# google-deepmind/mujoco_mpc

Measured on NVIDIA H100. Metric: env-steps/sec, higher is better.
Workload: dtype f32

## Files before the change

### mujoco_mpc_b200/csrc/dev_data.cuh

```cuda
#pragma once
#include <cuda_runtime.h>

#include "dev_model.h"

#ifndef MJPC_NO_COMPACT
#define MJPC_COMPACT 1
#endif
#ifdef MJPC_COMPACT
#define MJPC_ROLL _Pragma("unroll 1")
#define MJPC_HESS_ROLLED 1
#else
#define MJPC_ROLL
#endif

namespace mjpc_dev {

constexpr int kMaxSplinePoints = 64;
#define MJPC_D_ARRAYS(X)                                                                                          \
  X(qpos, M.nq) X(qvel, M.nv) X(ctrl, M.nu) X(qacc, M.nv) X(qacc_warmstart, M.nv) X(mocap_pos, 3 * M.nmocap)      \
  X(mocap_quat, 4 * M.nmocap) X(xpos, 3 * M.nbody) X(xquat, 4 * M.nbody) X(xmat, 9 * M.nbody)                     \
  X(xipos, 3 * M.nbody) X(ximat, 9 * M.nbody) X(xanchor, 3 * M.njnt) X(xaxis, 3 * M.njnt)                         \
  X(geom_xpos, 3 * M.ngeom) X(geom_xmat, 9 * M.ngeom) X(site_xpos, 3 * M.nsite) X(subtree_com, 3 * M.nbody)       \
  X(cinert, 10 * M.nbody) X(crb, 10 * M.nbody) X(cdof, 6 * M.nv) X(cdof_dot, 6 * M.nv) X(cvel, 6 * M.nbody)       \
  X(cacc, 6 * M.nbody) X(cfrc, 6 * M.nbody) X(cfrc_sub, 6 * M.nbody) X(subtree_linvel, 3 * M.nbody)               \
// ... 348 lines not shown
    y = mask_pick3(yj, lane == j, y - scaled * yj, lane > j, y, lane < j);
#pragma unroll
    for (int k = j + 1; k < N; k++) {
      const float lkj = __shfl_sync(kFull, row[j], k);
      row[k] -= row[j] * lkj;
    }
  }
  if (lane < N) {
#pragma unroll
    for (int k = 0; k < N; k++)
      if (k <= lane) A[lane * N + k] = row[k];
  }
  __syncwarp();
#pragma unroll
  for (int i = N - 1; i >= 0; i--) {
    const float xi = __shfl_sync(kFull, y, i) * il[i];
    if (lane == i) y = xi;
    if (lane < i) y -= A[i * N + lane] * xi;
  }
  if (lane < N) x[lane] = y;
  __syncwarp();
}

template <int N>
__device__ __forceinline__ void warp_chol_factor_solve_rolled(float* A, float* inv, float* x, const float* b, int lane) {
  const int li = lane < N ? lane : N - 1;
  float y = b[li];
  __syncwarp();
  float* rowi = A + li * N;
#pragma unroll 1
  for (int j = 0; j < N; j++) {
    const float* rowj = A + j * N;
    float s = rowi[j];
    int k = 0;
    if (N % 2 == 0) {
#pragma unroll 2
      for (; k + 1 < j; k += 2) {
        const float2 a = *reinterpret_cast<const float2*>(rowi + k), bb = *reinterpret_cast<const float2*>(rowj + k);
        s -= a.x * bb.x; s -= a.y * bb.y;
      }
    }
#pragma unroll 1
    for (; k < j; k++) s -= rowi[k] * rowj[k];
    float p = __shfl_sync(kFull, s, j);
    if (p < kMinVal) p = kMinVal;
    const float l = sqrtf(p), il = 1.0f / l;
    if (lane >= j && lane < N) rowi[j] = (lane == j) ? l : s * il;
    if (lane == j) inv[j] = il;
    __syncwarp();
  }
#pragma unroll 1
  for (int i = 0; i < N; i++) {
    const float yi = __shfl_sync(kFull, y, i) * inv[i];
    const float lij = rowi[i];
    y = (lane == i) ? yi : (lane > i ? y - lij * yi : y);
  }
#pragma unroll 1
  for (int i = N - 1; i >= 0; i--) {
    const float xi = __shfl_sync(kFull, y, i) * inv[i];
    const float lji = A[i * N + li];
    y = (lane == i) ? xi : (lane < i ? y - lji * xi : y);
  }
  if (lane < N) x[lane] = y;
  __syncwarp();
}

template <int NS>
__device__ __noinline__ void warp_chol_factor_solve(float* A, float* inv, float* x, const float* b, int n, int lane) {
#ifdef MJPC_CHOL_ROLLED2
  if constexpr (NS > 0 && NS <= 32) { warp_chol_factor_solve_rolled<NS>(A, inv, x, b, lane); return; }
  if (n == 18) { warp_chol_factor_solve_rolled<18>(A, inv, x, b, lane); return; }
#endif
#ifndef MJPC_CHOL_ROLLED
  if constexpr (NS > 0 && NS <= 32) { warp_chol_factor_solve_reg<NS>(A, x, b, lane); return; }
  if (n == 18) { warp_chol_factor_solve_reg<18>(A, x, b, lane); return; }
  if (n == 2) { warp_chol_factor_solve_reg<2>(A, x, b, lane); return; }
#endif
  warp_chol(A, inv, n, lane);
  warp_chol_solve(x, A, inv, b, n, lane);
}
#endif

}
```

### mujoco_mpc_b200/csrc/dev_model.h

```cpp
#pragma once
#include <cstdint>
#include <cstring>
#include <stdexcept>
#include <string>
#include <vector>

namespace mjpc_dev {

#define MJPC_F_ARRAYS(X)                                                                                         \
  X(body_pos) X(body_quat) X(body_ipos) X(body_iquat) X(body_mass) X(body_inertia) X(body_subtreemass)           \
  X(body_invweight0) X(jnt_pos) X(jnt_axis) X(jnt_range) X(jnt_stiffness) X(jnt_margin) X(jnt_solref)            \
  X(jnt_solimp) X(qpos0) X(qpos_spring) X(dof_damping) X(dof_armature) X(dof_frictionloss) X(dof_solref)         \
  X(dof_solimp) X(dof_invweight0) X(geom_size) X(geom_pos) X(geom_quat) X(geom_friction) X(geom_solmix)          \
  X(geom_solref) X(geom_solimp) X(geom_margin) X(geom_gap) X(geom_rbound) X(site_pos) X(site_quat)               \
  X(actuator_gear) X(actuator_gainprm) X(actuator_biasprm) X(actuator_ctrlrange) X(actuator_forcerange)          \
  X(key_qpos) X(task_weight) X(task_norm_parameter) X(task_parameters) X(task_state) X(wrap_coef) X(tendon_range)     \
  X(tendon_margin) X(tendon_solref) X(tendon_solimp) X(tendon_invweight0)
#define MJPC_I_ARRAYS(X)                                                                                         \
  X(body_parentid) X(body_rootid) X(body_jntnum) X(body_jntadr) X(body_dofnum) X(body_dofadr) X(body_mocapid)    \
  X(jnt_type) X(jnt_qposadr) X(jnt_dofadr) X(jnt_bodyid) X(jnt_limited) X(dof_bodyid) X(dof_jntid)               \
  X(dof_parentid) X(geom_type) X(geom_bodyid) X(geom_condim) X(geom_priority) X(site_bodyid) X(actuator_trnid) X(actuator_trntype)  \
  X(actuator_biastype) X(actuator_ctrllimited) X(actuator_forcelimited) X(pair_geom1) X(pair_geom2)              \
  X(ray_geoms) X(task_dim_norm_residual) X(task_norm) X(task_num_norm_parameter) X(task_trace_objtype)           \
  X(task_trace_objid) X(task_ids) X(tendon_adr) X(tendon_num) X(tendon_limited) X(wrap_dof) X(wrap_qposadr)
// ... 7 lines not shown
#undef X
      F_COUNT
};
enum IntArrayId {
#define X(n) I_##n,
  MJPC_I_ARRAYS(X) MJPC_I_DERIVED(X)
#undef X
      I_COUNT
};

enum { GEOM_PLANE = 0, GEOM_HFIELD, GEOM_SPHERE, GEOM_CAPSULE, GEOM_ELLIPSOID, GEOM_CYLINDER, GEOM_BOX };
enum { JNT_FREE = 0, JNT_BALL, JNT_SLIDE, JNT_HINGE };
enum { OBJ_BODY = 0, OBJ_XBODY, OBJ_GEOM, OBJ_SITE };
enum { CONE_PYRAMIDAL = 0, CONE_ELLIPTIC = 1 };
enum { RESIDUAL_PARTICLE = 0, RESIDUAL_PARTICLE_COPY = 1, RESIDUAL_CARTPOLE = 2, RESIDUAL_QUADRUPED_FLAT = 3,
       RESIDUAL_HUMANOID_STAND = 4, RESIDUAL_HUMANOID_TRACK = 5, RESIDUAL_SHADOW_REORIENT = 6 };

#define MJPC_M_INTS(X)                                                                                           \
  X(nq) X(nv) X(nu) X(nbody) X(njnt) X(ngeom) X(nsite) X(nmocap) X(nkey) X(npair) X(nray) X(nlevel) X(nmpair)    \
  X(ntendon)                                                                                                     \
  X(nfloss) X(nlimit) X(nhpair) X(cone) X(iterations) X(ls_iterations) X(disable_contact) X(disable_eulerdamp)  \
  X(disable_frictionloss) X(disable_limit) X(disable_refsafe) X(disable_warmstart) X(maxcon) X(maxefc)           \
  X(residual_id) X(num_residual) X(num_term) X(num_trace) X(num_parameters) X(task_state_size) X(any_damping)    \
  X(nf) X(ni)

struct DevModel {
#define X(n) int n;
  MJPC_M_INTS(X)
#undef X
  float timestep, impratio, tolerance, ls_tolerance, meaninertia, risk;
  float differentiable;
  float gravity[3];
  int fo[F_COUNT];
  int io[I_COUNT];
};

struct Blob {
  const uint8_t* p;
  size_t n;
  int nent;
  Blob(const void* data, size_t nbytes) : p((const uint8_t*)data), n(nbytes), nent(0) {
    if (!data || nbytes < 16 || std::memcmp(p, "MJPCB200", 8) != 0) throw std::runtime_error("bad model blob magic");
    std::memcpy(&nent, p + 12, 4);
    if ((size_t)16 + 56 * (size_t)nent > nbytes) throw std::runtime_error("truncated model blob");
  }
  bool find(const char* name, int* dt, int* cnt, int64_t* off) const {
    for (int i = 0; i < nent; i++) {
// ... 131 lines not shown
    std::vector<int> hi_, hj_, frow(nv, -1);
    for (int r = 0; r < nv; r++) for (int c2 = 0; c2 <= r; c2++) if (pat[(size_t)r * nv + c2]) { hi_.push_back(r); hj_.push_back(c2); }
    for (size_t k = 0; k < fl.size(); k++) frow[fl[k]] = (int)k;
    M.nhpair = (int)hi_.size();
    put(I_hpair_i, hi_); put(I_hpair_j, hj_); put(I_floss_row, frow);
    std::vector<int> cadr(nb, 0), cnum(nb, 0), cdofs;
    for (int bb = 0; bb < nb; bb++) {
      std::vector<int> ch;
      for (int d = lastdof[bb]; d >= 0; d = dofpar[d]) ch.push_back(d);
      cadr[bb] = (int)cdofs.size(); cnum[bb] = (int)ch.size();
      cdofs.insert(cdofs.end(), ch.rbegin(), ch.rend());
    }
    int widest = 0;
    for (size_t k = 0; k < g1.size(); k++) {
      const uint64_t c1 = chain(gb[g1[k]]), c2m = chain(gb[g2[k]]);
      const uint64_t mm = (c1 && c2m) ? (c1 ^ c2m) : (c1 | c2m);
      int cnt = 0;
      for (int r = 0; r < nv; r++) cnt += (int)((mm >> r) & 1);
      widest = std::max(widest, cnt);
    }
    if (widest > 16) throw std::runtime_error("a contact pair couples more than 16 dofs (compact Jacobian width)");
    put(I_chain_adr, cadr); put(I_chain_num, cnum); put(I_chain_dof, cdofs);
  }
  while (P.i.size() % 4) P.i.push_back(0);
  while (P.f.size() % 4) P.f.push_back(0.f);
  M.nf = (int)P.f.size(); M.ni = (int)P.i.size();
  return P;
}

}
```

### mujoco_mpc_b200/csrc/dev_physics.cuh

```cuda
#pragma once
#include "dev_data.cuh"

namespace mjpc_dev {



template <class SP>
__device__ __noinline__ void k_kinematics(Ctx& c) {
  auto&& M = SP::model(c);
  const int lane = c.lane;
  float *xpos = DF(xpos), *xquat = DF(xquat), *xmat = DF(xmat), *xipos = DF(xipos), *ximat = DF(ximat);
  float *xanchor = DF(xanchor), *xaxis = DF(xaxis);
  const float* qpos = DF(qpos);
  if (lane < 3) { xpos[lane] = 0; xipos[lane] = 0; }
  if (lane < 4) xquat[lane] = lane == 0 ? 1.f : 0.f;
  if (lane < 9) { float v = (lane % 4 == 0) ? 1.f : 0.f; xmat[lane] = v; ximat[lane] = v; }
  __syncwarp();
  const int *level_adr = MI(level_adr), *level_body = MI(level_body), *parentid = MI(body_parentid),
            *mocapid = MI(body_mocapid), *jntadr = MI(body_jntadr), *jntnum = MI(body_jntnum),
            *jtype = MI(jnt_type), *jqadr = MI(jnt_qposadr);
  const float *bpos = MF(body_pos), *bquat = MF(body_quat), *bipos = MF(body_ipos), *biquat = MF(body_iquat),
              *jpos = MF(jnt_pos), *jaxis = MF(jnt_axis), *qpos0 = MF(qpos0);
  for (int l = 0; l < M.nlevel; l++) {
    const int a = level_adr[l], e = level_adr[l + 1];
// ... 1014 lines not shown
  }
  __syncwarp();
  float* smooth = DF(qfrc_smooth);
  for (int i = lane; i < nv; i += 32) smooth[i] = passive[i] - bias[i] + qact[i];
  if (c.xfrc_on) {
    const float *xf = DF(xfrc), *cdof = DF(cdof), *xipos = DF(xipos), *scom = DF(subtree_com);
    const int *dbody = MI(dof_bodyid), *subend = MI(body_subtreeend), *rootid = MI(body_rootid);
    for (int i = lane; i < nv; i += 32) {
      const int b0 = dbody[i];
      const float* cd = cdof + 6 * i;
      float a = 0.f;
      MJPC_ROLL
      for (int b = b0; b < subend[b0]; b++) {
        float off[3], t[3];
        for (int q = 0; q < 3; q++) off[q] = xipos[3 * b + q] - scom[3 * rootid[b] + q];
        cross3(t, cd, off);
        const float* f = xf + 6 * b;
        for (int q = 0; q < 3; q++) a += (cd[3 + q] + t[q]) * f[q] + cd[q] * f[3 + q];
      }
      smooth[i] += a;
    }
  }
  __syncwarp();
  warp_chol_factor_solve<SP::kNV>(DF(qLD), DF(ldinv), DF(qacc_smooth), smooth, nv, lane);
}

template <class SP>
__device__ __noinline__ void k_reference(Ctx& c) {
  const int lane = c.lane;
  const float *qvel = DF(qvel), *K = DF(efc_K), *B = DF(efc_B), *imp = DF(efc_imp), *pos = DF(efc_pos),
              *margin = DF(efc_margin);
  float* aref = DF(efc_aref);
  const int nsimple = SP::model(c).nfloss + c.nlim;
  for (int i = lane; i < c.nefc; i += 32) {
    const float v = row_dot<SP>(c, i, nsimple, qvel);
    aref[i] = -B[i] * v - K[i] * imp[i] * (pos[i] - margin[i]);
  }
  __syncwarp();
}

template <class SP>
__device__ __noinline__ float k_update_constraint(Ctx& c, bool hess) {
  auto&& M = SP::model(c);
  const int lane = c.lane, nv = M.nv;
  const float *jar = DF(efc_jar), *D = DF(efc_D), *R = DF(efc_R), *floss = DF(efc_floss), *J = DF(efc_J);
  float *force = DF(efc_force), *X = DF(efc_W), *hw = DF(efc_hw), *xw = DF(efc_hc);
  int *state = DI(efc_state);
// ... 768 lines not shown
      const int i = min(b0 + lane, nv - 1);
      const bool on = b0 + lane < nv;
      const float a = Ma[i] - smooth[i] - qfc[i];
      if (on) grad[i] = a;
      g2 += on ? a * a : 0.f;
      const float m = fabsf(Ma[i]) + fabsf(smooth[i]) + fabsf(qfc[i]);
      ga += on ? m * m : 0.f;
    }
    const float gnorm2 = warp_sum(g2), gabs2 = warp_sum(ga);
    __syncwarp();
    if (iter > 0) {
      const float improvement = (old - cost) / scale_inv, gradient = sqrtf(gnorm2) / scale_inv;
      const float gfloor = kGradFloor * 1.1920929e-7f * sqrtf(gabs2) / scale_inv;
      if (gradient < fmaxf(tol, gfloor)) break;
      const bool resolvable = fabsf(old - cost) > 16.f * 1.1920929e-7f * fabsf(cost);
      if (resolvable) { if (improvement < tol) break; stalls = 0; }
      else if (gradient > 0.5f * prev_gradient && (alpha > 0.5f || ++stalls >= 3)) break;
      prev_gradient = gradient;
    }
    if (iter == M.iterations) break;
    PHASE(c, 4);
    k_hessian<SP>(c);
    PHASE(c, 5);
    warp_chol_factor_solve<SP::kNV>(DF(qH), DF(hinv), search, grad, nv, lane);
    PHASE(c, 6);
    for (int b0 = 0; b0 < nv; b0 += 32) { const int i = min(b0 + lane, nv - 1); const float v = -search[i]; __syncwarp(); if (b0 + lane < nv) search[i] = v; }
    __syncwarp();
    float q1 = 0, q2 = 0, sn = 0;
    for (int b0 = 0; b0 < nv; b0 += 32) {
      const int i = min(b0 + lane, nv - 1);
      const bool on = b0 + lane < nv;
      const float a = m_row_dot<SP>(qM, i, search, nv);
      if (on) Mv[i] = a;
      const float si = on ? search[i] : 0.f;
      q1 += si * (Ma[i] - smooth[i]);
      q2 += 0.5f * si * a;
      sn += si * si;
    }
    for (int b0 = 0; b0 < ne; b0 += 32) {
      const int i = min(b0 + lane, ne - 1);
      const float v = j_row_dot<SP>(c, i, nsimple, search, nv);
      if (b0 + lane < ne) Jv[i] = v;
    }
    q1 = warp_sum(q1); q2 = warp_sum(q2); sn = sqrtf(warp_sum(sn));
    __syncwarp();
    alpha = k_line_search<SP>(c, gauss, q1, q2, sn, scale_inv);
    if (alpha == 0.f) break;
// ... 29 lines not shown
  k_reference<SP>(c);
  PHASE(c, 3);
  k_solve<SP>(c);
  PHASE(c, 4);
}

template <class SP>
__device__ __noinline__ void k_euler(Ctx& c) {
  auto&& M = SP::model(c);
  const int lane = c.lane, nv = M.nv;
  const float h = CM(c).timestep;
  float *qacc = DF(qacc), *qvel = DF(qvel), *qpos = DF(qpos), *vt = DF(vtmp);
  const float* acc = qacc;
  if (M.any_damping && !M.disable_eulerdamp) {
    float *H = DF(qH), *qM = DF(qM), *smooth = DF(qfrc_smooth), *qfc = DF(qfrc_constraint);
    const float* damping = MF(dof_damping);
    MJPC_ROLL
    for (int w = lane; w < nv * nv; w += 32) {
      const int r = w / nv, s = w - r * nv;
      H[w] = qM[w] + (r == s ? h * damping[r] : 0.f);
    }
    for (int i = lane; i < nv; i += 32) vt[i] = smooth[i] + qfc[i];
    __syncwarp();
    warp_chol_factor_solve<SP::kNV>(H, DF(hinv), vt, vt, nv, lane);
    acc = vt;
  }
  for (int i = lane; i < nv; i += 32) qvel[i] += h * acc[i];
  __syncwarp();
  const int *jtype = MI(jnt_type), *jqadr = MI(jnt_qposadr), *jdadr = MI(jnt_dofadr);
  for (int j = lane; j < M.njnt; j += 32) {
    const int qa = jqadr[j], da = jdadr[j];
    const int t = jtype[j];
    if (t == JNT_FREE) {
      for (int q = 0; q < 3; q++) qpos[qa + q] += h * qvel[da + q];
      quat_integrate(qpos + qa + 3, qvel + da + 3, h);
    } else if (t == JNT_BALL) {
      quat_integrate(qpos + qa, qvel + da, h);
    } else {
      qpos[qa] += h * qvel[da];
    }
  }
  c.time += h;
  __syncwarp();
}

}
```

### mujoco_mpc_b200/csrc/engine.cu

```cuda
#include <cuda_runtime.h>
#include <dlfcn.h>
#include <nccl.h>

#include <algorithm>
#include <cmath>
#include <cstdio>
#include <cstdlib>
#include <cstring>
#include <string>
#include <vector>

#include "../../include/mjpc_b200.h"
#include "ilqg_kernels.cuh"
#include "rollout_kernels.cuh"

using namespace mjpc_dev;

namespace {
thread_local std::string g_last_error;
int fail(int code, const std::string& msg) { g_last_error = msg; return code; }

#define CUDA_TRY(expr)                                                                                     \
  do {                                                                                                     \
    cudaError_t e_ = (expr);                                                                               \
// ... 627 lines not shown
  if (M.task_state_size) CUDA_TRY(cudaMemcpy(h->d_task_state, ts.data(), ts.size() * 4, cudaMemcpyHostToDevice));
  DebugArgs A;
  std::memset(&A, 0, sizeof(A));
  A.M = h->pack.M; A.L = make_layout(h->pack.M, 1); A.pack = h->d_pack;
  A.qpos = d_qpos; A.qvel = d_qvel; A.ctrl = d_ctrl; A.mocap = d_mocap; A.warmstart = warmstart ? d_warm : nullptr;
  A.task_state = M.task_state_size ? h->d_task_state : nullptr;
  A.time = (float)time;
  A.qacc = d_qacc; A.residual = d_res; A.next_qpos = d_nq; A.next_qvel = d_nv; A.qM = d_qM; A.efc_force = d_force;
  A.counts = d_counts;
  step_debug_kernel<<<1, 32, h->smem_bytes(1, 1), h->stream>>>(A);
  h->launches += 1;
  CUDA_TRY(cudaGetLastError());
  CUDA_TRY(cudaStreamSynchronize(h->stream));
  if (qacc) CUDA_TRY(cudaMemcpy(qacc, d_qacc, nv * 4, cudaMemcpyDeviceToHost));
  if (residual) CUDA_TRY(cudaMemcpy(residual, d_res, nr * 4, cudaMemcpyDeviceToHost));
  if (next_qpos) CUDA_TRY(cudaMemcpy(next_qpos, d_nq, nq * 4, cudaMemcpyDeviceToHost));
  if (next_qvel) CUDA_TRY(cudaMemcpy(next_qvel, d_nv, nv * 4, cudaMemcpyDeviceToHost));
  if (qM) CUDA_TRY(cudaMemcpy(qM, d_qM, nv * nv * 4, cudaMemcpyDeviceToHost));
  if (efc_force) CUDA_TRY(cudaMemcpy(efc_force, d_force, 256 * 4, cudaMemcpyDeviceToHost));
  if (counts) CUDA_TRY(cudaMemcpy(counts, d_counts, 16, cudaMemcpyDeviceToHost));
  return 0;
}

int mjpc_b200_comm_unique_id(void* out, size_t nbytes) {
  if (!out || nbytes < sizeof(ncclUniqueId)) return fail(MJPC_B200_ERR_BAD_ARGUMENT, "comm_unique_id: need 128 bytes");
  NcclApi& api = nccl_api();
  if (!api.ok) return fail(MJPC_B200_ERR_UNSUPPORTED, "libnccl.so.2 not found");
  ncclUniqueId id;
  NCCL_TRY(api.GetUniqueId(&id));
  std::memcpy(out, &id, sizeof(id));
  return 0;
}

int mjpc_b200_comm_init(mjpc_b200_t* h, int nranks, int rank, const void* unique_id, size_t nbytes) {
  if (!h || nranks < 1 || rank < 0 || rank >= nranks || !unique_id || nbytes < sizeof(ncclUniqueId))
    return fail(MJPC_B200_ERR_BAD_ARGUMENT, "comm_init: bad argument");
  if (h->comm) return fail(MJPC_B200_ERR_BAD_ARGUMENT, "comm_init: communicator already initialised");
  NcclApi& api = nccl_api();
  if (!api.ok) return fail(MJPC_B200_ERR_UNSUPPORTED, "libnccl.so.2 not found");
  CUDA_TRY(cudaSetDevice(h->device));
  ncclUniqueId id;
  std::memcpy(&id, unique_id, sizeof(id));
  NCCL_TRY(api.CommInitRank(&h->comm, nranks, id, rank));
  h->nranks = nranks; h->rank = rank;
  h->maxTotal = nranks * h->maxN;
  const DevModel& M = h->pack.M;
// ... 315 lines not shown
```

### mujoco_mpc_b200/csrc/rollout_kernels.cuh

```cuda
#pragma once
#include "dev_physics.cuh"
#include "dev_task.cuh"
#include "spec_quadruped.h"
#include "spec_humanoid_track.h"

namespace mjpc_dev {

struct RolloutArgs {
  DevModel M;
  DevLayout L;
  const float* pack;
  int nprob, nper;
  const double* time0;
  const float* state;
  const float* mocap;
  const float* task_state;
  const float* weight;
  const float* parameters;
  const float* knots;
  const float* knot_times;
  FeedbackArgs fb;
  const float* step_sizes;
  int policy_kind;
  float xfrc_std, xfrc_rate;
// ... 344 lines not shown
  for (int i = lane; i < nq; i += 32) DF(qpos)[i] = A.qpos[i];
  for (int i = lane; i < nv; i += 32) { DF(qvel)[i] = A.qvel[i]; DF(qacc_warmstart)[i] = A.warmstart ? A.warmstart[i] : 0.f; }
  for (int i = lane; i < M.nu; i += 32) DF(ctrl)[i] = A.ctrl[i];
  for (int i = lane; i < 7 * M.nmocap; i += 32) {
    const int k = i / 7, q = i - 7 * k;
    if (q < 3) DF(mocap_pos)[3 * k + q] = A.mocap[i]; else DF(mocap_quat)[4 * k + q - 3] = A.mocap[i];
  }
  for (int i = lane; i < nv * nv; i += 32) DF(qM)[i] = 0;
  c.time = A.time;
  __syncwarp();
  k_forward<SP>(c);
  k_residual<SP>(c);
  if (k_bad(c, DF(qacc), nv)) c.warn = 1;
  for (int i = lane; i < nv; i += 32) A.qacc[i] = DF(qacc)[i];
  for (int i = lane; i < nv * nv; i += 32) A.qM[i] = DF(qM)[i];
  for (int i = lane; i < M.num_residual; i += 32) A.residual[i] = DF(residual)[i];
  for (int i = lane; i < c.nefc; i += 32) A.efc_force[i] = DF(efc_force)[i];
  if (lane == 0) { A.counts[0] = c.ncon - c.npseudo; A.counts[1] = c.nefc; A.counts[2] = c.niter; A.counts[3] = c.warn; }
  k_euler<SP>(c);
  for (int i = lane; i < nq; i += 32) A.next_qpos[i] = DF(qpos)[i];
  for (int i = lane; i < nv; i += 32) A.next_qvel[i] = DF(qvel)[i];
}


struct StepBatchArgs {
  DevModel M;
  DevLayout L;
  const float* pack;
  const float* qpos; const float* qvel; const float* ctrl; const float* warmstart;
  const float* mocap; const float* task_state;
  const float* time;
  int B;
  float* qacc; float* next_qpos; float* next_qvel; float* residual; float* cost; int* counts;
};

template <class SP>
__device__ __forceinline__ void step_batch_body(const StepBatchArgs& A) {
  float* smem = g_smem;
  stage_model_pack(smem, A.pack, (unsigned)((A.M.nf + A.M.ni) * 4));
  Ctx c;
  init_ctx(c, &A.M, &A.L, smem, 0, threadIdx.x, A.pack);
  auto&& M = SP::model(c);
  const int lane = c.lane, nq = M.nq, nv = M.nv, nu = M.nu, nr = M.num_residual;
  const int b = blockIdx.x;
  if (b >= A.B) return;
  if (A.task_state) {
// ... 44 lines not shown
```

### mujoco_mpc_b200/csrc/spec_humanoid_track.h

```cpp
#pragma once
namespace mjpc_dev {
struct SpecHumanoidTrack {
  static constexpr int kNumModelWords = 153;
  static constexpr int kNumLayout = 101;
  static constexpr int kModelWords[512] = {
      28, 27, 21, 37, 22, 20, 38, 16, 1889, 159, 20, 7, 243, 2, 0, 21,
      378, 0, 100, 50, 0, 0, 0, 0, 0, 0, 32, 96, 5, 141, 21, 1,
      0, 2, 1, 2604, 2900, 1000593162, 1065353216, 841731191, 1008981770, 1087545275, 0, 0, 0, 0, -1055066685, 0,
      112, 260, 372, 520, 560, 672, 712, 788, 856, 924, 968, 992, 1016, 1060, 1172, 1200,
      1228, 1256, 1284, 1312, 1368, 1504, 1532, 1592, 1652, 1732, 1792, 1812, 1852, 1952, 1972, 1992,
      2012, 2128, 2280, 2304, 2368, 2432, 2476, 2520, 2520, 2544, 2568, 2568, 2572, 2576, 2580, 2584,
      2588, 2600, 0, 37, 74, 111, 148, 185, 222, 259, 281, 303, 325, 347, 369, 396,
      423, 450, 470, 490, 510, 530, 568, 589, 610, 631, 652, 673, 832, 991, 1011, 1032,
      1053, 1074, 1075, 1076, 1108, 1110, 1112, 1114, 1118, 1122, 1130, 1166, 1203, 1240, 1277, 1314,
      1557, 1800, 1800, 1821, 2199, 2577, 2604, 2641, 2678, 0, 0, 0, 0, 0, 0, 0,
      0, 0, 0, 0, 0, 0, 0, 0, 0, 0, 0, 0, 0, 0, 0, 0,
      0, 0, 0, 0, 0, 0, 0, 0, 0, 0, 0, 0, 0, 0, 0, 0,
      0, 0, 0, 0, 0, 0, 0, 0, 0, 0, 0, 0, 0, 0, 0, 0,
      0, 0, 0, 0, 0, 0, 0, 0, 0, 0, 0, 0, 0, 0, 0, 0,
      0, 0, 0, 0, 0, 0, 0, 0, 0, 0, 0, 0, 0, 0, 0, 0,
      0, 0, 0, 0, 0, 0, 0, 0, 0, 0, 0, 0, 0, 0, 0, 0,
      0, 0, 0, 0, 0, 0, 0, 0, 0, 0, 0, 0, 0, 0, 0, 0,
      0, 0, 0, 0, 0, 0, 0, 0, 0, 0, 0, 0, 0, 0, 0, 0,
      0, 0, 0, 0, 0, 0, 0, 0, 0, 0, 0, 0, 0, 0, 0, 0,
      0, 0, 0, 0, 0, 0, 0, 0, 0, 0, 0, 0, 0, 0, 0, 0,
      0, 0, 0, 0, 0, 0, 0, 0, 0, 0, 0, 0, 0, 0, 0, 0,
      0, 0, 0, 0, 0, 0, 0, 0, 0, 0, 0, 0, 0, 0, 0, 0,
      0, 0, 0, 0, 0, 0, 0, 0, 0, 0, 0, 0, 0, 0, 0, 0,
      0, 0, 0, 0, 0, 0, 0, 0, 0, 0, 0, 0, 0, 0, 0, 0,
      0, 0, 0, 0, 0, 0, 0, 0, 0, 0, 0, 0, 0, 0, 0, 0,
      0, 0, 0, 0, 0, 0, 0, 0, 0, 0, 0, 0, 0, 0, 0, 0,
      0, 0, 0, 0, 0, 0, 0, 0, 0, 0, 0, 0, 0, 0, 0, 0,
      0, 0, 0, 0, 0, 0, 0, 0, 0, 0, 0, 0, 0, 0, 0, 0,
      0, 0, 0, 0, 0, 0, 0, 0, 0, 0, 0, 0, 0, 0, 0, 0,
      0, 0, 0, 0, 0, 0, 0, 0, 0, 0, 0, 0, 0, 0, 0, 0,
      0, 0, 0, 0, 0, 0, 0, 0, 0, 0, 0, 0, 0, 0, 0, 0,
      0, 0, 0, 0, 0, 0, 0, 0, 0, 0, 0, 0, 0, 0, 0, 0,
  };
// ... 21 lines not shown
```

### mujoco_mpc_b200/csrc/spec_quadruped.h

```cpp
#pragma once
namespace mjpc_dev {
struct SpecQuadruped {
  static constexpr int kNumModelWords = 153;
  static constexpr int kNumLayout = 101;
  static constexpr int kModelWords[512] = {
      19, 18, 12, 16, 13, 42, 6, 2, 2, 395, 4, 4, 117, 0, 12, 12,
      171, 1, 100, 50, 0, 0, 0, 0, 0, 0, 32, 96, 3, 42, 9, 1,
      11, 31, 1, 2124, 2144, 1008981770, 1092616192, 841731191, 1008981770, 1074405708, 0, 0, 0, 0, -1055066685, 0,
      48, 112, 160, 224, 240, 288, 304, 336, 376, 416, 444, 460, 476, 504, 572, 592,
      612, 632, 652, 672, 708, 800, 820, 948, 1076, 1244, 1372, 1416, 1500, 1712, 1756, 1800,
      1844, 1864, 1888, 1900, 1936, 1972, 1996, 2020, 2060, 2072, 2080, 2092, 2124, 2124, 2124, 2124,
      2124, 2124, 0, 16, 32, 48, 64, 80, 96, 112, 125, 138, 151, 164, 177, 195,
      213, 231, 273, 315, 357, 399, 405, 417, 429, 441, 453, 465, 860, 1255, 1259, 1268,
      1277, 1286, 1287, 1288, 1305, 1305, 1305, 1305, 1305, 1305, 1310, 1325, 1341, 1357, 1373, 1389,
      1506, 1623, 1635, 1647, 1818, 1989, 2007, 2023, 2039, 0, 0, 0, 0, 0, 0, 0,
      0, 0, 0, 0, 0, 0, 0, 0, 0, 0, 0, 0, 0, 0, 0, 0,
      0, 0, 0, 0, 0, 0, 0, 0, 0, 0, 0, 0, 0, 0, 0, 0,
      0, 0, 0, 0, 0, 0, 0, 0, 0, 0, 0, 0, 0, 0, 0, 0,
      0, 0, 0, 0, 0, 0, 0, 0, 0, 0, 0, 0, 0, 0, 0, 0,
      0, 0, 0, 0, 0, 0, 0, 0, 0, 0, 0, 0, 0, 0, 0, 0,
      0, 0, 0, 0, 0, 0, 0, 0, 0, 0, 0, 0, 0, 0, 0, 0,
      0, 0, 0, 0, 0, 0, 0, 0, 0, 0, 0, 0, 0, 0, 0, 0,
      0, 0, 0, 0, 0, 0, 0, 0, 0, 0, 0, 0, 0, 0, 0, 0,
      0, 0, 0, 0, 0, 0, 0, 0, 0, 0, 0, 0, 0, 0, 0, 0,
      0, 0, 0, 0, 0, 0, 0, 0, 0, 0, 0, 0, 0, 0, 0, 0,
      0, 0, 0, 0, 0, 0, 0, 0, 0, 0, 0, 0, 0, 0, 0, 0,
      0, 0, 0, 0, 0, 0, 0, 0, 0, 0, 0, 0, 0, 0, 0, 0,
      0, 0, 0, 0, 0, 0, 0, 0, 0, 0, 0, 0, 0, 0, 0, 0,
      0, 0, 0, 0, 0, 0, 0, 0, 0, 0, 0, 0, 0, 0, 0, 0,
      0, 0, 0, 0, 0, 0, 0, 0, 0, 0, 0, 0, 0, 0, 0, 0,
      0, 0, 0, 0, 0, 0, 0, 0, 0, 0, 0, 0, 0, 0, 0, 0,
      0, 0, 0, 0, 0, 0, 0, 0, 0, 0, 0, 0, 0, 0, 0, 0,
      0, 0, 0, 0, 0, 0, 0, 0, 0, 0, 0, 0, 0, 0, 0, 0,
      0, 0, 0, 0, 0, 0, 0, 0, 0, 0, 0, 0, 0, 0, 0, 0,
      0, 0, 0, 0, 0, 0, 0, 0, 0, 0, 0, 0, 0, 0, 0, 0,
      0, 0, 0, 0, 0, 0, 0, 0, 0, 0, 0, 0, 0, 0, 0, 0,
      0, 0, 0, 0, 0, 0, 0, 0, 0, 0, 0, 0, 0, 0, 0, 0,
  };
// ... 21 lines not shown
```

### mujoco_mpc_b200/engine.py

```python
from __future__ import annotations

import ctypes as C
import os

import numpy as np

from .blob import to_blob
from .build import SO

_fp = C.POINTER(C.c_float)
_dp = C.POINTER(C.c_double)
_ip = C.POINTER(C.c_int)
_bp = C.POINTER(C.c_uint8)

EXPORTS = ["mjpc_b200_version", "mjpc_b200_last_error", "mjpc_b200_create", "mjpc_b200_destroy",
           "mjpc_b200_get_info", "mjpc_b200_set_task", "mjpc_b200_set_differentiable", "mjpc_b200_set_xfrc_noise", "mjpc_b200_rollout_spline", "mjpc_b200_rollout_feedback",
           "mjpc_b200_rollout_spline_batched", "mjpc_b200_batch_planner_create", "mjpc_b200_batch_planner_destroy",
           "mjpc_b200_batch_planner_reset", "mjpc_b200_batch_planner_set_state", "mjpc_b200_batch_planner_set_task",
           "mjpc_b200_batch_planner_optimize_policy", "mjpc_b200_batch_planner_action_from_policy",
           "mjpc_b200_batch_planner_get_result",
           "mjpc_b200_fetch_trajectory", "mjpc_b200_fetch_all", "mjpc_b200_model_derivatives",
           "mjpc_b200_cost_derivatives", "mjpc_b200_backward_pass", "mjpc_b200_rollout_feedback_batched",
           "mjpc_b200_model_derivatives_batched", "mjpc_b200_cost_derivatives_batched", "mjpc_b200_backward_pass_batched",
           "mjpc_b200_batch_ilqg_planner_create", "mjpc_b200_batch_ilqg_planner_destroy",
# ... 343 lines not shown
        N, H = self.lastN, self.lastH
        o = dict(states=np.zeros((N, H, self.ds), np.float32), actions=np.zeros((N, H, self.nu), np.float32),
                 times=np.zeros((N, H)), residual=np.zeros((N, H, self.nr), np.float32),
                 costs=np.zeros((N, H), np.float32), trace=np.zeros((N, H, self.ntr), np.float32))
        self._check(self.lib.mjpc_b200_fetch_all(self.h, _pf(o["states"]), _pf(o["actions"]), _pd(o["times"]),
                                                 _pf(o["residual"]), _pf(o["costs"]), _pf(o["trace"])))
        return o

    def step_debug(self, qpos, qvel, ctrl, mocap, time=0.0, warmstart=None):
        nv, nq = self.info.nv, self.info.nq
        o = dict(qacc=np.zeros(nv, np.float32), residual=np.zeros(max(self.nr, 1), np.float32),
                 next_qpos=np.zeros(nq, np.float32), next_qvel=np.zeros(nv, np.float32),
                 qM=np.zeros((nv, nv), np.float32), efc_force=np.zeros(256, np.float32))
        counts = np.zeros(4, np.int32)
        q, v, u, mc, ws = _f(qpos), _f(qvel), _f(ctrl), _f(mocap), _f(warmstart)
        self._check(self.lib.mjpc_b200_step_debug(self.h, _pf(q), _pf(v), _pf(u), _pf(mc), C.c_double(time), _pf(ws),
                                                  _pf(o["qacc"]), _pf(o["residual"]), _pf(o["next_qpos"]),
                                                  _pf(o["next_qvel"]), _pf(o["qM"]), _pf(o["efc_force"]),
                                                  counts.ctypes.data_as(_ip)))
        o.update(ncon=int(counts[0]), nefc=int(counts[1]), niter=int(counts[2]), warning=int(counts[3]))
        o["efc_force"] = o["efc_force"][: o["nefc"]]
        return o

    def step_batch(self, qpos, qvel, ctrl, mocap, times, time0=0.0, warmstart=None):
        q, v, u, mc, ws, t = _f(qpos), _f(qvel), _f(ctrl), _f(mocap), _f(warmstart), _d(times)
        B, nv, nq = q.shape[0], self.info.nv, self.info.nq
        o = dict(qacc=np.zeros((B, nv), np.float32), next_qpos=np.zeros((B, nq), np.float32),
                 next_qvel=np.zeros((B, nv), np.float32), residual=np.zeros((B, max(self.nr, 1)), np.float32),
                 cost=np.zeros(B, np.float32))
        counts = np.zeros((B, 4), np.int32)
        self._check(self.lib.mjpc_b200_step_batch(self.h, B, _pf(q), _pf(v), _pf(u), _pf(ws), _pf(mc), C.c_double(time0),
                                                  _pd(t), _pf(o["qacc"]), _pf(o["next_qpos"]), _pf(o["next_qvel"]),
                                                  _pf(o["residual"]), _pf(o["cost"]), counts.ctypes.data_as(_ip)))
        o.update(ncon=counts[:, 0], nefc=counts[:, 1], niter=counts[:, 2], warning=counts[:, 3])
        return o

    def model_derivatives(self, x, u, t, mocap, tol, skip=0, mode=0):
        x, u, t, mc = _f(x), _f(u), _d(t), _f(mocap)
        H = x.shape[0]
        n, nu, nr = self.n, self.nu, self.nr
        A = np.zeros((H, n, n), np.float32); B = np.zeros((H, n, nu), np.float32)
        Cm = np.zeros((H, nr, n), np.float32); D = np.zeros((H, nr, nu), np.float32)
        self._check(self.lib.mjpc_b200_model_derivatives(self.h, _pf(x), _pf(u), _pd(t), _pf(mc), H, int(skip), C.c_float(tol), int(mode),
                                                         _pf(A), _pf(B), _pf(Cm), _pf(D)))
        return A, B, Cm, D

# ... 476 lines not shown
```

Measured before the change: 2.522 million.

## Add arrowhead block-sparse Cholesky solve for quadruped-shaped mass matrices

Detects at model build time whether the dof tree is a root chain followed by identical independent child chains (6 root, 4 legs of 3 for the quadruped). When it is, the warp Cholesky factor/solve uses a specialised arrowhead factorisation that handles the per-leg blocks in parallel across lanes and only does dense work on the root block. If any cross-leg coupling is nonzero it falls back to the dense register Cholesky. It also adds a debug kernel and host API to test the solver. The cost is extra register pressure, a warp-wide vote on every call, and more code in a noinline function.

```diff
diff --git a/mujoco_mpc_b200/csrc/dev_data.cuh b/mujoco_mpc_b200/csrc/dev_data.cuh
--- a/mujoco_mpc_b200/csrc/dev_data.cuh
+++ b/mujoco_mpc_b200/csrc/dev_data.cuh
@@ -394,6 +394,131 @@
   __syncwarp();
 }
 
+template <int R, int B, int S>
+__device__ __noinline__ int warp_arrow_factor_solve(float* A, float* x, const float* b, int lane) {
+  constexpr int BS = B * S, N = R + BS;
+  static_assert(N <= 32, "one row per lane");
+  const int li = lane < N ? lane : N - 1;
+  const bool child = li < BS;
+  const int cb = li / S, cm = li - S * (li / S);
+  const int orow = child ? R + li : li - BS;
+  float v[N];
+#pragma unroll
+  for (int k = 0; k < N; k++) v[k] = A[orow * N + (k < BS ? R + k : k - BS)];
+  float y = b[orow];
+  unsigned cross = 0;
+  float a[S];
+#pragma unroll
+  for (int k = 0; k < S; k++) a[k] = 0.f;
+#pragma unroll
+  for (int bb = 0; bb < B; bb++)
+#pragma unroll
+    for (int k = 0; k < S; k++) {
+      const bool mine = child && cb == bb;
+      a[k] = __int_as_float(__float_as_int(a[k]) | (__float_as_int(v[S * bb + k]) & (mine ? -1 : 0)));
+      cross |= (unsigned)__float_as_int(v[S * bb + k]) & ((child && !mine) ? 0x7fffffffu : 0u);
+    }
+  if (__any_sync(kFull, cross != 0u)) {
+    warp_chol_factor_solve_reg<N>(A, x, b, lane);
+    return 1;
+  }
+  __syncwarp();
+  float ilc[S];
+#pragma unroll
+  for (int k = 0; k < S; k++) {
+    float p = __shfl_sync(kFull, a[k], (S * cb + k) & 31);
+    if (p < kMinVal) p = kMinVal;
+    const float ilm = 1.0f / sqrtf(p);
+    float il[B], yk[B], ykm = 0.f;
+#pragma unroll
+    for (int bb = 0; bb < B; bb++) {
+      il[bb] = __shfl_sync(kFull, ilm, S * bb + k);
+      yk[bb] = __shfl_sync(kFull, y, S * bb + k) * il[bb];
+      ykm = mask_pick(yk[bb], cb == bb, ykm, cb != bb);
+    }
+    ilc[k] = ilm;
+    const float scaled = a[k] * ilm;
+    a[k] = scaled;
+    float ry = y;
+#pragma unroll
+    for (int bb = 0; bb < B; bb++) {
+      v[S * bb + k] *= il[bb];
+      ry -= v[S * bb + k] * yk[bb];
+    }
+    y = child ? mask_pick3(ykm, cm == k, y - scaled * ykm, cm > k, y, cm < k) : ry;
+#pragma unroll
+    for (int kk = k + 1; kk < S; kk++) {
+      float lm = 0.f;
+#pragma unroll
+      for (int bb = 0; bb < B; bb++) {
+        const float l = __shfl_sync(kFull, a[k], S * bb + kk);
+        lm = mask_pick(l, cb == bb, lm, cb != bb);
+        v[S * bb + kk] -= v[S * bb + k] * l;
+      }
+      a[kk] -= a[k] * lm;
+    }
+  }
+#pragma unroll
+  for (int p = 0; p < R; p++) {
+    float part[B];
+#pragma unroll
+    for (int bb = 0; bb < B; bb++) {
+      part[bb] = 0.f;
+#pragma unroll
+      for (int k = 0; k < S; k++) part[bb] += v[S * bb + k] * __shfl_sync(kFull, v[S * bb + k], BS + p);
+    }
+    float sum = part[0];
+#pragma unroll
+    for (int bb = 1; bb < B; bb++) sum += part[bb];
+    v[BS + p] -= sum;
+  }
+  float ilr[R];
+#pragma unroll
+  for (int j = BS; j < N; j++) {
+    float p = __shfl_sync(kFull, v[j], j);
+    if (p < kMinVal) p = kMinVal;
+    const float l = sqrtf(p);
+    ilr[j - BS] = 1.0f / l;
+    const float yj = __shfl_sync(kFull, y, j) * ilr[j - BS];
+    const float scaled = v[j] * ilr[j - BS];
+    v[j] = mask_pick(l, lane == j, scaled, lane != j);
+    y = mask_pick3(yj, lane == j, y - scaled * yj, lane > j, y, lane < j);
+#pragma unroll
+    for (int k = j + 1; k < N; k++) {
+      const float lkj = __shfl_sync(kFull, v[j], k);
+      v[k] -= v[j] * lkj;
+    }
+  }
+  if (lane < BS) {
+#pragma unroll
+    for (int k = 0; k < S; k++)
+      if (k <= cm) A[orow * N + R + S * cb + k] = a[k];
+  } else if (lane < N) {
+#pragma unroll
+    for (int j = 0; j < BS; j++) A[(R + j) * N + orow] = v[j];
+#pragma unroll
+    for (int k = 0; k < R; k++)
+      if (k <= orow) A[orow * N + k] = v[BS + k];
+  }
+  __syncwarp();
+#pragma unroll
+  for (int i = N - 1; i >= BS; i--) {
+    const int q = i - BS;
+    const float xi = __shfl_sync(kFull, y, i) * ilr[q];
+    const float lv = A[child ? (R + li) * N + q : q * N + orow];
+    y = mask_pick3(xi, lane == i, y - lv * xi, lane < i, y, lane > i);
+  }
+#pragma unroll
+  for (int k = S - 1; k >= 0; k--) {
+    const float xk = __shfl_sync(kFull, y, (S * cb + k) & 31) * ilc[k];
+    const float lv = A[child ? (R + S * cb + k) * N + R + S * cb + (cm < k ? cm : 0) : 0];
+    if (child) y = mask_pick3(xk, cm == k, y - lv * xk, cm < k, y, cm > k);
+  }
+  if (lane < N) x[orow] = y;
+  __syncwarp();
+  return 0;
+}
+
 template <int N>
 __device__ __forceinline__ void warp_chol_factor_solve_rolled(float* A, float* inv, float* x, const float* b, int lane) {
   const int li = lane < N ? lane : N - 1;
@@ -437,20 +562,24 @@
   __syncwarp();
 }
 
+template <class MM>
+__device__ __forceinline__ bool arrow_643(const MM& M) { return M.blk_root == 6 && M.blk_nchild == 4 && M.blk_size == 3; }
 template <int NS>
-__device__ __noinline__ void warp_chol_factor_solve(float* A, float* inv, float* x, const float* b, int n, int lane) {
+__device__ __noinline__ int warp_chol_factor_solve(float* A, float* inv, float* x, const float* b, int n, int lane, bool arrow) {
+  if (arrow) return warp_arrow_factor_solve<6, 4, 3>(A, x, b, lane);
 #ifdef MJPC_CHOL_ROLLED2
-  if constexpr (NS > 0 && NS <= 32) { warp_chol_factor_solve_rolled<NS>(A, inv, x, b, lane); return; }
-  if (n == 18) { warp_chol_factor_solve_rolled<18>(A, inv, x, b, lane); return; }
+  if constexpr (NS > 0 && NS <= 32) { warp_chol_factor_solve_rolled<NS>(A, inv, x, b, lane); return 1; }
+  if (n == 18) { warp_chol_factor_solve_rolled<18>(A, inv, x, b, lane); return 1; }
 #endif
 #ifndef MJPC_CHOL_ROLLED
-  if constexpr (NS > 0 && NS <= 32) { warp_chol_factor_solve_reg<NS>(A, x, b, lane); return; }
-  if (n == 18) { warp_chol_factor_solve_reg<18>(A, x, b, lane); return; }
-  if (n == 2) { warp_chol_factor_solve_reg<2>(A, x, b, lane); return; }
+  if constexpr (NS > 0 && NS <= 32) { warp_chol_factor_solve_reg<NS>(A, x, b, lane); return 1; }
+  if (n == 18) { warp_chol_factor_solve_reg<18>(A, x, b, lane); return 1; }
+  if (n == 2) { warp_chol_factor_solve_reg<2>(A, x, b, lane); return 1; }
 #endif
   warp_chol(A, inv, n, lane);
   warp_chol_solve(x, A, inv, b, n, lane);
-}
-#endif
-
-}
+  return 1;
+}
+#endif
+
+}
diff --git a/mujoco_mpc_b200/csrc/dev_model.h b/mujoco_mpc_b200/csrc/dev_model.h
--- a/mujoco_mpc_b200/csrc/dev_model.h
+++ b/mujoco_mpc_b200/csrc/dev_model.h
@@ -53,7 +53,7 @@
   X(nfloss) X(nlimit) X(nhpair) X(cone) X(iterations) X(ls_iterations) X(disable_contact) X(disable_eulerdamp)  \
   X(disable_frictionloss) X(disable_limit) X(disable_refsafe) X(disable_warmstart) X(maxcon) X(maxefc)           \
   X(residual_id) X(num_residual) X(num_term) X(num_trace) X(num_parameters) X(task_state_size) X(any_damping)    \
-  X(nf) X(ni)
+  X(blk_root) X(blk_nchild) X(blk_size) X(nf) X(ni)
 
 struct DevModel {
 #define X(n) int n;
@@ -231,6 +231,22 @@
     if (widest > 16) throw std::runtime_error("a contact pair couples more than 16 dofs (compact Jacobian width)");
     put(I_chain_adr, cadr); put(I_chain_num, cnum); put(I_chain_dof, cdofs);
   }
+  {
+    std::vector<int> nchild(nv, 0);
+    for (int d = 1; d < nv; d++) if (dofpar[d] >= 0) nchild[dofpar[d]]++;
+    int r = 0;
+    while (r < nv && dofpar[r] == r - 1 && nchild[r] == 1) r++;
+    M.blk_root = M.blk_nchild = M.blk_size = 0;
+    if (r < nv && dofpar[r] == r - 1 && nchild[r] > 1) {
+      const int root = r + 1, nb2 = nchild[r], size = (nv - root) / nb2;
+      bool ok = size > 0 && root + nb2 * size == nv;
+      for (int d = root; ok && d < nv; d++) {
+        const int k = (d - root) % size;
+        ok = (k == 0 ? dofpar[d] == r : dofpar[d] == d - 1) && nchild[d] == (k + 1 < size ? 1 : 0);
+      }
+      if (ok) { M.blk_root = root; M.blk_nchild = nb2; M.blk_size = size; }
+    }
+  }
   while (P.i.size() % 4) P.i.push_back(0);
   while (P.f.size() % 4) P.f.push_back(0.f);
   M.nf = (int)P.f.size(); M.ni = (int)P.i.size();
diff --git a/mujoco_mpc_b200/csrc/dev_physics.cuh b/mujoco_mpc_b200/csrc/dev_physics.cuh
--- a/mujoco_mpc_b200/csrc/dev_physics.cuh
+++ b/mujoco_mpc_b200/csrc/dev_physics.cuh
@@ -1060,7 +1060,7 @@
     }
   }
   __syncwarp();
-  warp_chol_factor_solve<SP::kNV>(DF(qLD), DF(ldinv), DF(qacc_smooth), smooth, nv, lane);
+  warp_chol_factor_solve<SP::kNV>(DF(qLD), DF(ldinv), DF(qacc_smooth), smooth, nv, lane, arrow_643(M));
 }
 
 template <class SP>
@@ -1875,7 +1875,7 @@
     PHASE(c, 4);
     k_hessian<SP>(c);
     PHASE(c, 5);
-    warp_chol_factor_solve<SP::kNV>(DF(qH), DF(hinv), search, grad, nv, lane);
+    warp_chol_factor_solve<SP::kNV>(DF(qH), DF(hinv), search, grad, nv, lane, arrow_643(M));
     PHASE(c, 6);
     for (int b0 = 0; b0 < nv; b0 += 32) { const int i = min(b0 + lane, nv - 1); const float v = -search[i]; __syncwarp(); if (b0 + lane < nv) search[i] = v; }
     __syncwarp();
@@ -1951,7 +1951,7 @@
     }
     for (int i = lane; i < nv; i += 32) vt[i] = smooth[i] + qfc[i];
     __syncwarp();
-    warp_chol_factor_solve<SP::kNV>(H, DF(hinv), vt, vt, nv, lane);
+    warp_chol_factor_solve<SP::kNV>(H, DF(hinv), vt, vt, nv, lane, arrow_643(M));
     acc = vt;
   }
   for (int i = lane; i < nv; i += 32) qvel[i] += h * acc[i];
diff --git a/mujoco_mpc_b200/csrc/engine.cu b/mujoco_mpc_b200/csrc/engine.cu
--- a/mujoco_mpc_b200/csrc/engine.cu
+++ b/mujoco_mpc_b200/csrc/engine.cu
@@ -673,6 +673,29 @@
   return 0;
 }
 
+extern "C" int mjpc_b200_debug_factor_solve(mjpc_b200_t* h, int count, const float* A, const float* b, float* x, int* dense) {
+  if (!h || count < 1 || !A || !b || !x || !dense) return fail(MJPC_B200_ERR_BAD_ARGUMENT, "debug_factor_solve: bad argument");
+  const DevModel& M = h->pack.M;
+  const size_t n = M.nv;
+  CUDA_TRY(cudaSetDevice(h->device));
+  float *dA = nullptr, *db = nullptr, *dx = nullptr;
+  int* dd = nullptr;
+  CUDA_TRY(cudaMalloc(&dA, count * n * n * 4));
+  CUDA_TRY(cudaMalloc(&db, count * n * 4));
+  CUDA_TRY(cudaMalloc(&dx, count * n * 4));
+  CUDA_TRY(cudaMalloc(&dd, count * 4));
+  CUDA_TRY(cudaMemcpy(dA, A, count * n * n * 4, cudaMemcpyHostToDevice));
+  CUDA_TRY(cudaMemcpy(db, b, count * n * 4, cudaMemcpyHostToDevice));
+  factor_debug_kernel<<<count, 32, (n * n + 2 * n) * 4, h->stream>>>(M, dA, db, dx, dd);
+  h->launches += 1;
+  CUDA_TRY(cudaGetLastError());
+  CUDA_TRY(cudaStreamSynchronize(h->stream));
+  CUDA_TRY(cudaMemcpy(x, dx, count * n * 4, cudaMemcpyDeviceToHost));
+  CUDA_TRY(cudaMemcpy(dense, dd, count * 4, cudaMemcpyDeviceToHost));
+  cudaFree(dA); cudaFree(db); cudaFree(dx); cudaFree(dd);
+  return 0;
+}
+
 int mjpc_b200_comm_unique_id(void* out, size_t nbytes) {
   if (!out || nbytes < sizeof(ncclUniqueId)) return fail(MJPC_B200_ERR_BAD_ARGUMENT, "comm_unique_id: need 128 bytes");
   NcclApi& api = nccl_api();
diff --git a/mujoco_mpc_b200/csrc/rollout_kernels.cuh b/mujoco_mpc_b200/csrc/rollout_kernels.cuh
--- a/mujoco_mpc_b200/csrc/rollout_kernels.cuh
+++ b/mujoco_mpc_b200/csrc/rollout_kernels.cuh
@@ -390,6 +390,20 @@
   for (int i = lane; i < nv; i += 32) A.next_qvel[i] = DF(qvel)[i];
 }
 
+extern "C" __global__ void __launch_bounds__(32) factor_debug_kernel(const __grid_constant__ DevModel M, const float* A,
+                                                                     const float* b, float* x, int* dense) {
+  extern __shared__ __align__(16) float smem[];
+  const int n = M.nv, lane = threadIdx.x;
+  const size_t k = blockIdx.x;
+  float *a = smem, *v = smem + n * n, *inv = v + n;
+  for (int i = lane; i < n * n; i += 32) a[i] = A[k * n * n + i];
+  for (int i = lane; i < n; i += 32) v[i] = b[k * n + i];
+  __syncwarp();
+  const int d = warp_chol_factor_solve<0>(a, inv, v, v, n, lane, arrow_643(M));
+  for (int i = lane; i < n; i += 32) x[k * n + i] = v[i];
+  if (lane == 0) dense[k] = d;
+}
+
 
 struct StepBatchArgs {
   DevModel M;
diff --git a/mujoco_mpc_b200/csrc/spec_humanoid_track.h b/mujoco_mpc_b200/csrc/spec_humanoid_track.h
--- a/mujoco_mpc_b200/csrc/spec_humanoid_track.h
+++ b/mujoco_mpc_b200/csrc/spec_humanoid_track.h
@@ -1,19 +1,19 @@
 #pragma once
 namespace mjpc_dev {
 struct SpecHumanoidTrack {
-  static constexpr int kNumModelWords = 153;
+  static constexpr int kNumModelWords = 156;
   static constexpr int kNumLayout = 101;
   static constexpr int kModelWords[512] = {
       28, 27, 21, 37, 22, 20, 38, 16, 1889, 159, 20, 7, 243, 2, 0, 21,
       378, 0, 100, 50, 0, 0, 0, 0, 0, 0, 32, 96, 5, 141, 21, 1,
-      0, 2, 1, 2604, 2900, 1000593162, 1065353216, 841731191, 1008981770, 1087545275, 0, 0, 0, 0, -1055066685, 0,
-      112, 260, 372, 520, 560, 672, 712, 788, 856, 924, 968, 992, 1016, 1060, 1172, 1200,
-      1228, 1256, 1284, 1312, 1368, 1504, 1532, 1592, 1652, 1732, 1792, 1812, 1852, 1952, 1972, 1992,
-      2012, 2128, 2280, 2304, 2368, 2432, 2476, 2520, 2520, 2544, 2568, 2568, 2572, 2576, 2580, 2584,
-      2588, 2600, 0, 37, 74, 111, 148, 185, 222, 259, 281, 303, 325, 347, 369, 396,
-      423, 450, 470, 490, 510, 530, 568, 589, 610, 631, 652, 673, 832, 991, 1011, 1032,
-      1053, 1074, 1075, 1076, 1108, 1110, 1112, 1114, 1118, 1122, 1130, 1166, 1203, 1240, 1277, 1314,
-      1557, 1800, 1800, 1821, 2199, 2577, 2604, 2641, 2678, 0, 0, 0, 0, 0, 0, 0,
+      0, 2, 1, 0, 0, 0, 2604, 2900, 1000593162, 1065353216, 841731191, 1008981770, 1087545275, 0, 0, 0,
+      0, -1055066685, 0, 112, 260, 372, 520, 560, 672, 712, 788, 856, 924, 968, 992, 1016,
+      1060, 1172, 1200, 1228, 1256, 1284, 1312, 1368, 1504, 1532, 1592, 1652, 1732, 1792, 1812, 1852,
+      1952, 1972, 1992, 2012, 2128, 2280, 2304, 2368, 2432, 2476, 2520, 2520, 2544, 2568, 2568, 2572,
+      2576, 2580, 2584, 2588, 2600, 0, 37, 74, 111, 148, 185, 222, 259, 281, 303, 325,
+      347, 369, 396, 423, 450, 470, 490, 510, 530, 568, 589, 610, 631, 652, 673, 832,
+      991, 1011, 1032, 1053, 1074, 1075, 1076, 1108, 1110, 1112, 1114, 1118, 1122, 1130, 1166, 1203,
+      1240, 1277, 1314, 1557, 1800, 1800, 1821, 2199, 2577, 2604, 2641, 2678, 0, 0, 0, 0,
       0, 0, 0, 0, 0, 0, 0, 0, 0, 0, 0, 0, 0, 0, 0, 0,
       0, 0, 0, 0, 0, 0, 0, 0, 0, 0, 0, 0, 0, 0, 0, 0,
       0, 0, 0, 0, 0, 0, 0, 0, 0, 0, 0, 0, 0, 0, 0, 0,
diff --git a/mujoco_mpc_b200/csrc/spec_quadruped.h b/mujoco_mpc_b200/csrc/spec_quadruped.h
--- a/mujoco_mpc_b200/csrc/spec_quadruped.h
+++ b/mujoco_mpc_b200/csrc/spec_quadruped.h
@@ -1,19 +1,19 @@
 #pragma once
 namespace mjpc_dev {
 struct SpecQuadruped {
-  static constexpr int kNumModelWords = 153;
+  static constexpr int kNumModelWords = 156;
   static constexpr int kNumLayout = 101;
   static constexpr int kModelWords[512] = {
       19, 18, 12, 16, 13, 42, 6, 2, 2, 395, 4, 4, 117, 0, 12, 12,
       171, 1, 100, 50, 0, 0, 0, 0, 0, 0, 32, 96, 3, 42, 9, 1,
-      11, 31, 1, 2124, 2144, 1008981770, 1092616192, 841731191, 1008981770, 1074405708, 0, 0, 0, 0, -1055066685, 0,
-      48, 112, 160, 224, 240, 288, 304, 336, 376, 416, 444, 460, 476, 504, 572, 592,
-      612, 632, 652, 672, 708, 800, 820, 948, 1076, 1244, 1372, 1416, 1500, 1712, 1756, 1800,
-      1844, 1864, 1888, 1900, 1936, 1972, 1996, 2020, 2060, 2072, 2080, 2092, 2124, 2124, 2124, 2124,
-      2124, 2124, 0, 16, 32, 48, 64, 80, 96, 112, 125, 138, 151, 164, 177, 195,
-      213, 231, 273, 315, 357, 399, 405, 417, 429, 441, 453, 465, 860, 1255, 1259, 1268,
-      1277, 1286, 1287, 1288, 1305, 1305, 1305, 1305, 1305, 1305, 1310, 1325, 1341, 1357, 1373, 1389,
-      1506, 1623, 1635, 1647, 1818, 1989, 2007, 2023, 2039, 0, 0, 0, 0, 0, 0, 0,
+      11, 31, 1, 6, 4, 3, 2124, 2144, 1008981770, 1092616192, 841731191, 1008981770, 1074405708, 0, 0, 0,
+      0, -1055066685, 0, 48, 112, 160, 224, 240, 288, 304, 336, 376, 416, 444, 460, 476,
+      504, 572, 592, 612, 632, 652, 672, 708, 800, 820, 948, 1076, 1244, 1372, 1416, 1500,
+      1712, 1756, 1800, 1844, 1864, 1888, 1900, 1936, 1972, 1996, 2020, 2060, 2072, 2080, 2092, 2124,
+      2124, 2124, 2124, 2124, 2124, 0, 16, 32, 48, 64, 80, 96, 112, 125, 138, 151,
+      164, 177, 195, 213, 231, 273, 315, 357, 399, 405, 417, 429, 441, 453, 465, 860,
+      1255, 1259, 1268, 1277, 1286, 1287, 1288, 1305, 1305, 1305, 1305, 1305, 1305, 1310, 1325, 1341,
+      1357, 1373, 1389, 1506, 1623, 1635, 1647, 1818, 1989, 2007, 2023, 2039, 0, 0, 0, 0,
       0, 0, 0, 0, 0, 0, 0, 0, 0, 0, 0, 0, 0, 0, 0, 0,
       0, 0, 0, 0, 0, 0, 0, 0, 0, 0, 0, 0, 0, 0, 0, 0,
       0, 0, 0, 0, 0, 0, 0, 0, 0, 0, 0, 0, 0, 0, 0, 0,
diff --git a/mujoco_mpc_b200/engine.py b/mujoco_mpc_b200/engine.py
--- a/mujoco_mpc_b200/engine.py
+++ b/mujoco_mpc_b200/engine.py
@@ -389,6 +389,13 @@
         o["efc_force"] = o["efc_force"][: o["nefc"]]
         return o
 
+    def debug_factor_solve(self, A, b):
+        a, bb = _f(A), _f(b)
+        K = bb.shape[0]
+        x, dense = np.zeros_like(bb), np.zeros(K, np.int32)
+        self._check(self.lib.mjpc_b200_debug_factor_solve(self.h, K, _pf(a), _pf(bb), _pf(x), dense.ctypes.data_as(_ip)))
+        return x, dense.astype(bool)
+
     def step_batch(self, qpos, qvel, ctrl, mocap, times, time0=0.0, warmstart=None):
         q, v, u, mc, ws, t = _f(qpos), _f(qvel), _f(ctrl), _f(mocap), _f(warmstart), _d(times)
         B, nv, nq = q.shape[0], self.info.nv, self.info.nq
```

After: 2.550 million (median of 6 runs). 1.01x the previous value.
